# yisol/IDM-VTON

Measured on AMD Instinct MI355X. Metric: try-on images/sec at 768x1024, 30 DDIM steps, guidance 2.0, higher is better.
Workload: dtype bf16; 1 GPU; BASELINE.json configs[1]: 768x1024, 30 steps, batch 2/GPU, guidance 2.0, bf16 storage / fp32 accumulate, scheduler ddim, hipGraph on, GarmentNet batched over 6 timesteps, GarmentNet(block b+1)||TryonNet(block b) two-stream overlap on; images_per_call=2, parallelism=dp1 (image shards, one start-up RCCL weight broadcast), rccl_ranks=1

## Files before the change

### idm-vton_amd/csrc/gemm_body.cuh

```cuda
#pragma once
#include <type_traits>
#if !defined(__gfx950__) && !defined(__gfx942__) && defined(__HIP_DEVICE_COMPILE__)
#error "gemm_body.cuh: the counted vmcnt pipeline is written for gfx94x/gfx950 (stores counted in vmcnt)"
#endif
#include "common.cuh"
#include "gemm_common.cuh"

template <typename T, int BN, int BM, int WN, int WM, int ST, bool V1, bool LIN, bool PF, bool TR, bool XA = false>
__device__ __forceinline__ void gemm_body(const GemmParams& p, char* smem, const int m0, const int n0) {
    typedef typename VT<T>::v8 v8;
    typedef typename VT<T>::v4 v4;
    constexpr int NW = WN * WM;
    constexpr int SN = BN / WN, SM = BM / WM;
    constexpr int NI = SN / 32, MI = SM / 32;
    constexpr int WBYTES = BN * 128, XBYTES = BM * 128;
    constexpr int PW_ = BN / 8, PX_ = BM / 8;
    constexpr bool UNEVEN = (PW_ % NW != 0) || (PX_ % NW != 0);
    constexpr int WI = (PW_ + NW - 1) / NW, XI = (PX_ + NW - 1) / NW;
    static_assert(BN % 8 == 0 && BM % 8 == 0 && WN * SN == BN && WM * SM == BM && NI * 32 == SN && MI * 32 == SM, "tile / wave-count mismatch");
    static_assert(!UNEVEN || (V1 && ST == 2), "round-robin piece assignment needs the two-stage ring");
    char* sW = smem;
    char* sX = smem + ST * WBYTES;

    const int lane = threadIdx.x & 63;
// ... 56 lines not shown
            for (int i = 0; i < XI; ++i) {
                if (UNEVEN && xj(i) >= PX_) continue;
                int iy = x_oy[i] + sg.dy, ix = x_ox[i] + sg.dx;
                const bool ok = (unsigned)iy < (unsigned)hin && (unsigned)ix < (unsigned)win;
                if (p.ups) { iy >>= 1; ix >>= 1; }
                const uint32_t off = ((uint32_t)(x_pix[i] + iy * p.Wi + ix) * (uint32_t)sg.pitch + sg.coff + kseg + x_c8[i]) * 2u;
                dma16(rs_x, dX + xj(i) * 1024, ok ? off : OOB_SENTINEL);
            }
            kseg += 64;
            if (kseg >= sg.len) { kseg = 0; ++si; }
        }
    };

    idmvton_seg sgc = p.seg[0];
    __amdgpu_buffer_rsrc_t rs_xc = rs_x0;
    auto issue_part = [&](int t, int buf, int s) {
        constexpr int LPT_ = WI + XI;
        char* dW = sW + buf * WBYTES;
        char* dX = sX + buf * XBYTES;
        if constexpr (!LIN) {
            if (s == 0) { sgc = p.seg[si]; rs_xc = make_rsrc(sgc.ptr, sgc.bytes); }
        }
#pragma unroll
        for (int j = 0; j < LPT_; ++j) {
            if ((j & 3) != s) continue;
            if (j < WI) {
                if (UNEVEN && wj(j) >= PW_) continue;
                dma16(rs_w, dW + wj(j) * 1024, w_off[j] + kbyte(t));
            } else {
                const int i = j - WI;
                if (UNEVEN && xj(i) >= PX_) continue;
                if constexpr (LIN) dma16(rs_x0, dX + xj(i) * 1024, x_off[i] + kbyte(t));
                else {
                    int iy = x_oy[i] + sgc.dy, ix = x_ox[i] + sgc.dx;
                    const bool ok = (unsigned)iy < (unsigned)hin && (unsigned)ix < (unsigned)win;
                    if (p.ups) { iy >>= 1; ix >>= 1; }
                    const uint32_t off = ((uint32_t)(x_pix[i] + iy * p.Wi + ix) * (uint32_t)sgc.pitch + sgc.coff + kseg + x_c8[i]) * 2u;
                    dma16(rs_xc, dX + xj(i) * 1024, ok ? off : OOB_SENTINEL);
                }
            }
        }
        if constexpr (!LIN) {
            if (s == 3) { kseg += 64; if (kseg >= sgc.len) { kseg = 0; ++si; } }
        }
    };

    int a_row[NI], a_swz[NI], b_row[MI], b_swz[MI];
#pragma unroll
    for (int ni = 0; ni < NI; ++ni) { const int r = wn * SN + ni * 32 + l31; a_row[ni] = r * 128; a_swz[ni] = (r >> 1) & 7; }
#pragma unroll
    for (int mi = 0; mi < MI; ++mi) { const int r = wm * SM + mi * 32 + l31; b_row[mi] = r * 128; b_swz[mi] = (r >> 1) & 7; }

    f32x16 acc[NI][MI];
#pragma unroll
    for (int ni = 0; ni < NI; ++ni)
#pragma unroll
        for (int mi = 0; mi < MI; ++mi)
#pragma unroll
            for (int r = 0; r < 16; ++r) acc[ni][mi][r] = 0.f;

    auto frag_a = [&](const char* bW, int s, int ni) { return *(const v8*)(bW + a_row[ni] + (((2 * s + u) ^ a_swz[ni]) << 4)); };
    auto frag_b = [&](const char* bX, int s, int mi) { return *(const v8*)(bX + b_row[mi] + (((2 * s + u) ^ b_swz[mi]) << 4)); };
    auto compute = [&](int buf, bool spread = false, int t_next = 0, int buf_next = 0) {
        const char* bW = sW + buf * WBYTES;
        const char* bX = sX + buf * XBYTES;
        if constexpr (!PF) {
#pragma unroll
            for (int s = 0; s < 4; ++s) {
                v8 a[NI], b[MI];
#pragma unroll
                for (int ni = 0; ni < NI; ++ni) a[ni] = frag_a(bW, s, ni);
#pragma unroll
                for (int mi = 0; mi < MI; ++mi) b[mi] = frag_b(bX, s, mi);
                if constexpr (V1) {
                    if (spread) issue_part(t_next, buf_next, s);
                    __builtin_amdgcn_sched_barrier(0);
                }
#pragma unroll
                for (int ni = 0; ni < NI; ++ni)
#pragma unroll
                    for (int mi = 0; mi < MI; ++mi)
                        acc[ni][mi] = TR ? VT<T>::mfma(b[mi], a[ni], acc[ni][mi]) : VT<T>::mfma(a[ni], b[mi], acc[ni][mi]);
            }
        } else {
            v8 a[2][NI], b[2][MI];
#pragma unroll
            for (int ni = 0; ni < NI; ++ni) a[0][ni] = frag_a(bW, 0, ni);
#pragma unroll
            for (int mi = 0; mi < MI; ++mi) b[0][mi] = frag_b(bX, 0, mi);
#pragma unroll
            for (int s = 0; s < 4; ++s) {
                if (s < 3) {
#pragma unroll
                    for (int ni = 0; ni < NI; ++ni) a[(s + 1) & 1][ni] = frag_a(bW, s + 1, ni);
#pragma unroll
                    for (int mi = 0; mi < MI; ++mi) b[(s + 1) & 1][mi] = frag_b(bX, s + 1, mi);
                }
                if (spread) issue_part(t_next, buf_next, s);
                __builtin_amdgcn_sched_barrier(0);
#pragma unroll
                for (int ni = 0; ni < NI; ++ni)
#pragma unroll
                    for (int mi = 0; mi < MI; ++mi)
                        acc[ni][mi] = TR ? VT<T>::mfma(b[s & 1][mi], a[s & 1][ni], acc[ni][mi])
                                         : VT<T>::mfma(a[s & 1][ni], b[s & 1][mi], acc[ni][mi]);
                __builtin_amdgcn_sched_barrier(0);
            }
        }
    };

    v8 xkf[XA ? XA_NK : 1];
    int xa_b = 0, xa_h = 0;
    if constexpr (XA) {
        static_assert(NI == 2 && !TR, "fused cross-attention: one 64-channel head per wave");
        const int mw = m0 + wm * SM;
        xa_b = (mw < p.M ? mw : p.M - 1) / p.xa.tokens;
        xa_h = (n0 + wn * SN) >> 6;
        xattn_load_k<T>(p.xa, xa_b, xa_h, lane, xkf);
    }
    const int nt = p.Ktot >> 6;
    if constexpr (!V1) {
        issue(0, 0);
        for (int t = 0; t < nt; ++t) {
            asm volatile("s_waitcnt vmcnt(0)" ::: "memory");
            __syncthreads();
            if (t + 1 < nt) issue(t + 1, (t + 1) & 1);
            compute(t & 1);
        }
    } else {
        constexpr int LPT = WI + XI;
        static_assert((ST - 2) * LPT < 64, "vmcnt immediate is 6 bits");
#pragma unroll
        for (int s = 0; s < ST - 1; ++s)
            if (s < nt) issue(s, s);
        int cbuf = 0, ibuf = ST - 1;
        for (int t = 0; t < nt; ++t) {
            if (t + ST - 2 < nt) wait_vmcnt<(ST - 2) * LPT>(); else wait_vmcnt<0>();
            __builtin_amdgcn_s_barrier();
            asm volatile("" ::: "memory");
            compute(cbuf, t + ST - 1 < nt, t + ST - 1, ibuf);
            cbuf = cbuf + 1 == ST ? 0 : cbuf + 1;
            ibuf = ibuf + 1 == ST ? 0 : ibuf + 1;
        }
    }

    if constexpr (XA) {
        v8 xvf[XA_NV];
        xattn_load_v<T>(p.xa, xa_b, xa_h, lane, xvf);
        xattn_compute<T, MI>(p.xa, p.M, acc, m0 + wm * SM, lane, xkf, xvf);
    }
    gemm_epilogue<T, NI, MI, SN, SM, TR>(p, acc, m0, n0, wn, wm, lane);
}

template <typename T, int BN, int BM, int WN, int WM, int ST, bool V1, bool LIN, int OCC, bool PFX = false>
__global__ __launch_bounds__(WN * WM * 64, OCC) void gemm_conv_kernel(const GemmParams p) {
    __shared__ __attribute__((aligned(1024))) char smem[ST * (BN + BM) * 128];
    const int wg = xcd_remap(blockIdx.x, p.tiles_m * p.tiles_n);
    int tm, tn;
    if constexpr (!V1) { tm = wg / p.tiles_n; tn = wg - tm * p.tiles_n; }
    else {
        const int GM = p.gm > 0 ? p.gm : 1024 / BM;
        const int width = GM * p.tiles_n;
        const int grp = wg / width, rem = wg - grp * width;
        const int first = grp * GM;
        const int gsz = p.tiles_m - first < GM ? p.tiles_m - first : GM;
        tn = rem / gsz; tm = first + (rem - tn * gsz);
    }
    const int m0 = tm * BM, n0 = tn * BN;
    if constexpr (BN == 320) {
        gemm_body<T, BN, BM, WN, WM, ST, V1, LIN, OCC == 1 || PFX, false>(p, smem, m0, n0);
    } else {
        if (p.vt != nullptr && n0 >= p.vt_n0) gemm_body<T, BN, BM, WN, WM, ST, V1, LIN, OCC == 1 || PFX, true>(p, smem, m0, n0);
        else gemm_body<T, BN, BM, WN, WM, ST, V1, LIN, OCC == 1 || PFX, false>(p, smem, m0, n0);
    }
}

template <typename T, int BN, int BM, int WN, int WM, int ST, int OCC>
__global__ __launch_bounds__(WN * WM * 64, OCC) void gemm_xattn_kernel(const GemmParams p) {
    __shared__ __attribute__((aligned(1024))) char smem[ST * (BN + BM) * 128];
    const int wg = xcd_remap(blockIdx.x, p.tiles_m * p.tiles_n);
    const int GM = p.gm > 0 ? p.gm : 1024 / BM;
    const int width = GM * p.tiles_n;
    const int grp = wg / width, rem = wg - grp * width;
    const int first = grp * GM;
    const int gsz = p.tiles_m - first < GM ? p.tiles_m - first : GM;
    const int tn = rem / gsz, tm = first + (rem - tn * gsz);
    gemm_body<T, BN, BM, WN, WM, ST, true, true, OCC == 1, false, true>(p, smem, tm * BM, tn * BN);
}

template <typename T, int BN, int BM, int WN, int WM, int ST, bool V1, int OCC, bool PFX = false>
static void launch_cfg(const GemmParams& p0, bool lin, hipStream_t st) {
    GemmParams p = p0;
    p.gm = V1 ? idmvton_choose_gm(p.tiles_m, p.tiles_n, BM, BN, p.Ktot) : 0;
    const dim3 grid(p.tiles_n * p.tiles_m), block(WN * WM * 64);
    if constexpr (V1) {
        if (lin) { hipLaunchKernelGGL((gemm_conv_kernel<T, BN, BM, WN, WM, ST, true, true, OCC, PFX>), grid, block, 0, st, p); return; }
    }
    hipLaunchKernelGGL((gemm_conv_kernel<T, BN, BM, WN, WM, ST, V1, false, OCC, PFX>), grid, block, 0, st, p);
}


int gemm_tiles_v0(const GemmParams& p, bool bf16, int bn, int bm, bool lin, hipStream_t st);
int gemm_tiles_v1(const GemmParams& p, bool bf16, int bn, int bm, bool lin, hipStream_t st);
int gemm_tiles_v2(const GemmParams& p, bool bf16, int bn, int bm, bool lin, hipStream_t st);
int gemm_tiles_w8(const GemmParams& p, bool bf16, int bn, int bm, int form, bool lin, hipStream_t st);
int gemm_tiles_xattn(const GemmParams& p, bool bf16, int bn, int bm, int w8, hipStream_t st);
int launch_gemm_lin(const GemmParams& p, bool bf16, int bm, int form, int grid_cap, hipStream_t st);
```

### idm-vton_amd/csrc/gemm_common.cuh

```cuda
#pragma once
#include "common.cuh"
#include "xattn.cuh"

struct GemmParams {
    const void* w; uint32_t w_bytes; int N; int Ktot;
    int nseg; idmvton_seg seg[IDMVTON_MAX_SEG];
    int M, Ho, Wo, Hi, Wi, stride, ups;
    void* out; int ldo;
    const void* bias; const void* rowbias; int rowbias_ld; int rows_per_group;
    const void* res; int ldr;
    int mode;
    void* vt; int vt_n0; int vt_tokens; int vt_perm;
    int colscale_n; float colscale;
    int tiles_m, tiles_n;
    int gm;
    int wide;
    int res32, out32;
    int bias32;
    int out8; float o8_scale, vt8_scale;
    XAttnParams xa;
};

int idmvton_choose_gm(int tiles_m, int tiles_n, int bm, int bn, int K);

template <int N> __device__ __forceinline__ void wait_vmcnt() { asm volatile("s_waitcnt vmcnt(%0)" ::"n"(N) : "memory"); }

__device__ __forceinline__ void swap_cols8(const f32x16& c, const int gp, float (&v)[8]) {
#pragma unroll
    for (int j = 0; j < 4; ++j) {
        const auto r = __builtin_amdgcn_permlane32_swap(__float_as_uint(c[8 * gp + j]), __float_as_uint(c[8 * gp + 4 + j]), false, false);
        v[j] = __uint_as_float(r[0]);
        v[4 + j] = __uint_as_float(r[1]);
    }
}

template <typename T, int NI, int MI, int SN, int SM, bool TR>
__device__ __forceinline__ void gemm_epilogue(const GemmParams& p, f32x16 (&acc)[NI][MI], const int m0, const int n0, const int wn, const int wm,
                                              const int lane) {
    typedef typename VT<T>::v4 v4;
    typedef typename VT<T>::v8 v8;
    const int u = lane >> 5, l31 = lane & 31;
    const T* bias = (const T*)p.bias;
    if constexpr (TR) {
        if (p.out8) {
            uint8_t* vt = (uint8_t*)p.vt;
            const int Cv = p.N - p.vt_n0;
#pragma unroll
            for (int ni = 0; ni < NI; ++ni) {
                const int n = n0 + wn * SN + ni * 32 + l31;
                if (n >= p.N) continue;
                const float bv = bias ? (float)bias[n] : 0.f;
#pragma unroll
                for (int mi = 0; mi < MI; ++mi) {
                    const int m = m0 + wm * SM + mi * 32;
                    if (m >= p.M) continue;
                    const int b = m / p.vt_tokens;
                    const int tok = m - b * p.vt_tokens;
                    int4 o;
                    int w[4];
#pragma unroll
                    for (int g = 0; g < 4; ++g)
                        w[g] = pack4_fp8(clamp448((acc[ni][mi][4 * g] + bv) * p.vt8_scale), clamp448((acc[ni][mi][4 * g + 1] + bv) * p.vt8_scale),
                                         clamp448((acc[ni][mi][4 * g + 2] + bv) * p.vt8_scale), clamp448((acc[ni][mi][4 * g + 3] + bv) * p.vt8_scale));
                    o.x = w[0]; o.y = w[1]; o.z = w[2]; o.w = w[3];
                    *(int4*)(vt + ((size_t)(b * Cv + n - p.vt_n0) * p.vt_tokens + (tok & ~63) + 32 * u + ((tok >> 1) & 16))) = o;
                }
            }
            return;
        }
        if (p.vt_perm) {
            T* vt = (T*)p.vt;
            const int Cv = p.N - p.vt_n0;
#pragma unroll
            for (int ni = 0; ni < NI; ++ni) {
                const int n = n0 + wn * SN + ni * 32 + l31;
                if (n >= p.N) continue;
                const float bv = bias ? (float)bias[n] : 0.f;
#pragma unroll
                for (int mi = 0; mi < MI; ++mi)
#pragma unroll
                    for (int gp = 0; gp < 2; ++gp) {
                        const int m = m0 + wm * SM + mi * 32 + 16 * gp;
                        if (m >= p.M) continue;
                        const int b = m / p.vt_tokens;
                        const int tok = m - b * p.vt_tokens + 8 * u;
                        v8 o;
#pragma unroll
                        for (int j = 0; j < 8; ++j) o[j] = (T)(acc[ni][mi][8 * gp + j] + bv);
                        *(v8*)(vt + ((size_t)(b * Cv + n - p.vt_n0) * p.vt_tokens + tok)) = o;
                    }
            }
            return;
        }
        T* vt = (T*)p.vt;
        const int Cv = p.N - p.vt_n0;
#pragma unroll
        for (int ni = 0; ni < NI; ++ni) {
            const int n = n0 + wn * SN + ni * 32 + l31;
            if (n >= p.N) continue;
            const float bv = bias ? (float)bias[n] : 0.f;
#pragma unroll
            for (int mi = 0; mi < MI; ++mi)
#pragma unroll
                for (int g = 0; g < 4; ++g) {
                    const int m = m0 + wm * SM + mi * 32 + 8 * g + 4 * u;
                    if (m >= p.M) continue;
                    const int b = m / p.vt_tokens;
                    int tok = m - b * p.vt_tokens;
                    if (p.vt_perm) tok = (tok & ~12) | ((tok & 4) << 1) | ((tok & 8) >> 1);
                    v4 o;
#pragma unroll
                    for (int j = 0; j < 4; ++j) o[j] = (T)(acc[ni][mi][4 * g + j] + bv);
                    *(v4*)(vt + ((size_t)(b * Cv + n - p.vt_n0) * p.vt_tokens + tok)) = o;
                }
        }
        return;
    }
    T* out = (T*)p.out;
    const T* res = (const T*)p.res;
    const T* rowbias = (const T*)p.rowbias;
    if (p.wide) {
#pragma unroll
        for (int mi = 0; mi < MI; ++mi) {
            const int m = m0 + wm * SM + mi * 32 + l31;
            if (m >= p.M) continue;
            const T* rb = rowbias ? rowbias + (size_t)(m / p.rows_per_group) * p.rowbias_ld : nullptr;
            if (p.mode == IDMVTON_EPI_GEGLU) {
                if constexpr (NI % 2 == 0) {
#pragma unroll
                    for (int pr = 0; pr < NI / 2; ++pr)
#pragma unroll
                        for (int gp = 0; gp < 2; ++gp) {
                            float h[8], gt[8];
                            swap_cols8(acc[2 * pr][mi], gp, h);
                            swap_cols8(acc[2 * pr + 1][mi], gp, gt);
                            const int nh = n0 + wn * SN + pr * 64 + 16 * gp + 8 * u;
                            if (nh + 32 >= p.N) continue;
                            const int jo = ((n0 + wn * SN + pr * 64) >> 1) + 16 * gp + 8 * u;
                            if (bias) {
                                const v8 bh = *(const v8*)(bias + nh), bg = *(const v8*)(bias + nh + 32);
#pragma unroll
                                for (int j = 0; j < 8; ++j) { h[j] += (float)bh[j]; gt[j] += (float)bg[j]; }
                            }
                            v8 o;
#pragma unroll
                            for (int j = 0; j < 8; ++j) o[j] = (T)(h[j] * gelu_erf(gt[j]));
                            *(v8*)(out + (size_t)m * p.ldo + jo) = o;
                        }
                }
                continue;
            }
#pragma unroll
            for (int ni = 0; ni < NI; ++ni) {
#pragma unroll
                for (int gp = 0; gp < 2; ++gp) {
                    float v[8];
                    swap_cols8(acc[ni][mi], gp, v);
                    const int n = n0 + wn * SN + ni * 32 + 16 * gp + 8 * u;
                    if (n >= p.N) continue;
                    if (bias) {
                        if (p.bias32) {
                            const float4* bp = (const float4*)((const float*)p.bias + n);
                            const float4 b0 = bp[0], b1 = bp[1];
                            v[0] += b0.x; v[1] += b0.y; v[2] += b0.z; v[3] += b0.w;
                            v[4] += b1.x; v[5] += b1.y; v[6] += b1.z; v[7] += b1.w;
                        } else {
                            const v8 bb = *(const v8*)(bias + n);
#pragma unroll
                            for (int j = 0; j < 8; ++j) v[j] += (float)bb[j];
                        }
                    }
                    if (rb) {
// ... 120 lines not shown
```

### idm-vton_amd/csrc/gemm_conv.hip

```cpp
#include <cstdlib>
#include <cstring>
#include <vector>
#include "gemm_body.cuh"

int launch_gemm_lin(const GemmParams& p, bool bf16, int bm, int form, int grid_cap, hipStream_t st);

#include <map>
#include <mutex>
#include <tuple>
int idmvton_choose_gm(int tiles_m, int tiles_n, int bm, int bn, int K) {
    static const char* env = getenv("IDMVTON_GM");
    if (env) return atoi(env);
    static const bool model = getenv("IDMVTON_GM_MODEL") && atoi(getenv("IDMVTON_GM_MODEL")) != 0;
    if (!model) return 0;
    static std::mutex mu;
    static std::map<std::tuple<int, int, int, int, int>, int> cache;
    const auto key = std::make_tuple(tiles_m, tiles_n, bm, bn, K);
    std::lock_guard<std::mutex> lk(mu);
    auto it = cache.find(key);
    if (it != cache.end()) return it->second;
    const int T = tiles_m * tiles_n, q = T / 8, r = T % 8;
    static const long cap = getenv("IDMVTON_GM_CAP_KB") ? atol(getenv("IDMVTON_GM_CAP_KB")) << 10 : (2l << 20);
    long best = -1; int best_gm = 0;
    for (int gm = 1; gm <= tiles_m; ++gm) {
// ... 12 lines not shown
                if (!ns[tn]) { ns[tn] = 1; ++cn; }
            }
            (void)m_lo; (void)m_hi;
            cost += (long)cm * bm + (long)cn * bn;
        }
        if (best < 0 || cost < best) { best = cost; best_gm = gm; }
    }
    cache[key] = best_gm;
    return best_gm;
}

static int launch_gemm(const GemmParams& p0, bool bf16, int variant, int bn, int bm, bool lin, hipStream_t st) {
    GemmParams p = p0;
    int form = 0;
    int grid_cap = 0;
    if (variant == 5) { form = bm & 15; grid_cap = (bm & 0x4000) ? 5 : 0; bm &= ~(15 | 0x4000); }
    p.tiles_n = (p.N + bn - 1) / bn;
    p.tiles_m = (p.M + bm - 1) / bm;
    int rc = 1;
    if (p.mode == IDMVTON_EPI_XATTN) {
        if (bm != 64 && p.xa.tokens % 64 != 0) {
            bm = 64;
            p.tiles_m = (p.M + bm - 1) / bm;
        }
        if (gemm_tiles_xattn(p, bf16, bn, bm, variant == 6 && bn == 128 && bm == 128, st))
            return idmvton_set_error(IDMVTON_E_ARG, "gemm_conv: IDMVTON_EPI_XATTN runs on the 128x64, 128x128 and 128x256 tiles (got %dx%d)", bn, bm);
        CHECK_LAUNCH("gemm_conv");
        return IDMVTON_OK;
    }
    if (variant == 0) rc = gemm_tiles_v0(p, bf16, bn, bm, lin, st);
    else if (variant == 1) rc = gemm_tiles_v1(p, bf16, bn, bm, lin, st);
    else if (variant == 2) rc = gemm_tiles_v2(p, bf16, bn, bm, lin, st);
    else if (variant == 5) {
        if (!(bn == 256 && (bm == 256 || bm == 192))) return idmvton_set_error(IDMVTON_E_ARG, "gemm_conv: variant 5 is the 256x256 / 256x192 tile");
        if (lin) rc = launch_gemm_lin(p, bf16, bm, form, grid_cap, st);
        else if (bm == 256) rc = gemm_tiles_v1(p, bf16, 256, 256, lin, st);
        else {
            p.tiles_n = (p.N + 127) / 128; p.tiles_m = (p.M + 255) / 256;
            rc = gemm_tiles_v1(p, bf16, 128, 256, lin, st);
        }
    } else if (variant == 6) {
        const int form6 = bm & 15;
        bm &= ~15;
        p.tiles_m = (p.M + bm - 1) / bm;
        if (bn == 320 && (p.vt || !p.wide || p.out8 || p.mode == IDMVTON_EPI_GEGLU)) {
            const int fbn = bn == 320 ? 128 : bn, fbm = bn == 320 ? 256 : bm;
            p.tiles_n = (p.N + fbn - 1) / fbn;
            p.tiles_m = (p.M + fbm - 1) / fbm;
            rc = gemm_tiles_v1(p, bf16, fbn, fbm, lin, st);
        } else rc = gemm_tiles_w8(p, bf16, bn, bm, form6, lin, st);
    } else return idmvton_set_error(IDMVTON_E_ARG, "gemm_conv: unknown variant %d", variant);
    if (rc) return idmvton_set_error(IDMVTON_E_ARG, "gemm_conv: variant %d has no %dx%d tile", variant, bn, bm);
    CHECK_LAUNCH("gemm_conv");
    return IDMVTON_OK;
}

extern "C" int idmvton_gemm_conv(const idmvton_gemm_conv_args* a, void* stream) {
    CHECK_ARG(a != nullptr, IDMVTON_E_ARG, "gemm_conv: null args");
    CHECK_ARG(a->dtype == IDMVTON_F16 || a->dtype == IDMVTON_BF16, IDMVTON_E_DTYPE, "gemm_conv: dtype %d", a->dtype);
    CHECK_ARG(a->M > 0 && a->N > 0 && a->Ktot > 0, IDMVTON_E_SHAPE, "gemm_conv: M=%d N=%d K=%d", a->M, a->N, a->Ktot);
    CHECK_ARG(a->Ktot % 64 == 0, IDMVTON_E_SHAPE, "gemm_conv: Ktot=%d must be a multiple of 64", a->Ktot);
    CHECK_ARG(a->N % 4 == 0, IDMVTON_E_SHAPE, "gemm_conv: N=%d must be a multiple of 4", a->N);
    CHECK_ARG(a->nseg >= 1 && a->nseg <= IDMVTON_MAX_SEG, IDMVTON_E_SHAPE, "gemm_conv: nseg=%d", a->nseg);
    int ksum = 0;
    for (int s = 0; s < a->nseg; ++s) {
        const idmvton_seg& g = a->seg[s];
        CHECK_ARG(g.ptr && g.len > 0 && g.len % 64 == 0, IDMVTON_E_SHAPE, "gemm_conv: seg %d len=%d", s, g.len);
        CHECK_ARG(g.pitch % 8 == 0 && g.coff % 8 == 0, IDMVTON_E_ALIGN, "gemm_conv: seg %d pitch=%d coff=%d", s, g.pitch, g.coff);
        CHECK_ARG(g.bytes < 0x80000000u, IDMVTON_E_SHAPE, "gemm_conv: seg %d tensor >= 2 GiB", s);
        CHECK_ARG(((uintptr_t)g.ptr & 15) == 0, IDMVTON_E_ALIGN, "gemm_conv: seg %d pointer not 16-byte aligned", s);
        ksum += g.len;
    }
    CHECK_ARG(ksum == a->Ktot, IDMVTON_E_SHAPE, "gemm_conv: segment lengths sum to %d, Ktot=%d", ksum, a->Ktot);
    CHECK_ARG(a->Ho > 0 && a->Wo > 0 && a->Hi > 0 && a->Wi > 0 && a->stride > 0 && a->M % (a->Ho * a->Wo) == 0,
              IDMVTON_E_SHAPE, "gemm_conv: geometry M=%d Ho=%d Wo=%d", a->M, a->Ho, a->Wo);
    if (a->ups) CHECK_ARG(a->stride == 1 && a->Ho <= 2 * a->Hi && a->Ho >= 2 * a->Hi - 1 && a->Wo <= 2 * a->Wi && a->Wo >= 2 * a->Wi - 1, IDMVTON_E_SHAPE,
                          "gemm_conv: ups=1 needs stride 1 and an output grid of 2Hi x 2Wi or one short of it (Ho=%d Hi=%d Wo=%d Wi=%d)", a->Ho, a->Hi, a->Wo, a->Wi);
    CHECK_ARG(a->w && ((uintptr_t)a->w & 15) == 0, IDMVTON_E_ALIGN, "gemm_conv: weight pointer");
    const uint64_t wbytes = (uint64_t)a->N * a->Ktot * 2;
    CHECK_ARG(wbytes + (uint64_t)128 * a->Ktot * 2 < 0xFFFFFFFFull, IDMVTON_E_SHAPE, "gemm_conv: weight too large");
    const bool geglu = a->mode == IDMVTON_EPI_GEGLU, xattn = a->mode == IDMVTON_EPI_XATTN;
    CHECK_ARG(a->mode == IDMVTON_EPI_NONE || a->mode == IDMVTON_EPI_GELU || a->mode == IDMVTON_EPI_QUICKGELU || geglu || xattn, IDMVTON_E_ARG, "gemm_conv: mode %d", a->mode);
    CHECK_ARG(a->colscale_n >= 0 && a->colscale_n % 4 == 0 && !(geglu && a->colscale_n), IDMVTON_E_ARG, "gemm_conv: colscale_n=%d", a->colscale_n);
    if (geglu) CHECK_ARG(a->N % 64 == 0 && !a->res && !a->rowbias && !a->vt, IDMVTON_E_ARG, "gemm_conv: GEGLU needs N%%64==0, no res/rowbias/vt");
    CHECK_ARG(a->out || (a->vt && a->vt_n0 == 0), IDMVTON_E_ARG, "gemm_conv: null out");
    if (a->out) CHECK_ARG(a->ldo % 4 == 0 && ((uintptr_t)a->out & 7) == 0, IDMVTON_E_ALIGN, "gemm_conv: out alignment");
    if (a->res) CHECK_ARG(a->ldr % 4 == 0 && ((uintptr_t)a->res & 7) == 0, IDMVTON_E_ALIGN, "gemm_conv: res alignment");
    if (a->bias) CHECK_ARG(((uintptr_t)a->bias & 7) == 0, IDMVTON_E_ALIGN, "gemm_conv: bias alignment");
    if (a->rowbias) CHECK_ARG(a->rowbias_ld % 4 == 0 && a->rows_per_group > 0 && ((uintptr_t)a->rowbias & 7) == 0,
                              IDMVTON_E_ALIGN, "gemm_conv: rowbias");
    if (a->vt && a->vt_perm) CHECK_ARG(((uintptr_t)a->vt & 15) == 0, IDMVTON_E_ALIGN, "gemm_conv: vt pointer not 16-byte aligned");
    if (a->vt && a->vt_perm) CHECK_ARG(a->vt_tokens % 16 == 0, IDMVTON_E_ARG, "gemm_conv: vt_perm needs vt_tokens %% 16 == 0 (got %d)", a->vt_tokens);
    if (a->vt) CHECK_ARG(a->vt_tokens > 0 && a->vt_tokens % 4 == 0 && a->M % a->vt_tokens == 0 && a->vt_n0 % 64 == 0 &&
                         a->vt_n0 >= 0 && a->vt_n0 < a->N && ((uintptr_t)a->vt & 7) == 0,
                         IDMVTON_E_ARG, "gemm_conv: vt_tokens=%d vt_n0=%d", a->vt_tokens, a->vt_n0);

    GemmParams p;
    memset(&p.xa, 0, sizeof(p.xa));
    if (xattn) {
        const idmvton_xattn* x = a->xattn;
        CHECK_ARG(x != nullptr && (x->nseg == 1 || x->nseg == 2), IDMVTON_E_ARG, "gemm_conv: IDMVTON_EPI_XATTN needs `xattn` with 1 or 2 key segments");
        CHECK_ARG(a->N % 64 == 0 && !a->bias && !a->res && !a->rowbias && !a->vt && !a->colscale_n && !a->io_flags &&
                  a->nseg == 1 && a->Ho == 1 && a->Hi == 1 && a->Wo == a->M && a->Wi == a->M && a->out && a->ldo % 8 == 0 && ((uintptr_t)a->out & 15) == 0,
                  IDMVTON_E_ARG, "gemm_conv: IDMVTON_EPI_XATTN is a plain Linear with N %% 64 == 0 and nothing else in its epilogue");
        CHECK_ARG(x->tokens > 0 && x->tokens % 32 == 0 && a->M % x->tokens == 0, IDMVTON_E_SHAPE, "gemm_conv: xattn.tokens=%d (rows per batch element, a multiple of 32 dividing M=%d)", x->tokens, a->M);
        for (int s = 0; s < x->nseg; ++s) {
            const int nk_max = s == 0 ? 96 : 32;
            CHECK_ARG(x->k[s] && x->vt[s] && x->nk[s] > 0 && x->nk[s] <= nk_max && x->k_rows[s] >= ((x->nk[s] + 31) & ~31) && x->ldk[s] >= a->N && x->ldk[s] % 8 == 0 &&
                      x->ldvt[s] >= ((x->nk[s] + 15) & ~15) && x->ldvt[s] % 8 == 0 && (((uintptr_t)x->k[s] | (uintptr_t)x->vt[s]) & 15) == 0, IDMVTON_E_SHAPE,
                      "gemm_conv: xattn segment %d: nk=%d (<= %d) k_rows=%d (>= round32(nk)) ldk=%d ldvt=%d (>= round16(nk))", s, x->nk[s], nk_max, x->k_rows[s], x->ldk[s], x->ldvt[s]);
            p.xa.k[s] = x->k[s]; p.xa.vt[s] = x->vt[s]; p.xa.ldk[s] = x->ldk[s]; p.xa.ldvt[s] = x->ldvt[s]; p.xa.nk[s] = x->nk[s]; p.xa.krows[s] = x->k_rows[s];
        }
        p.xa.nseg = x->nseg; p.xa.tokens = x->tokens; p.xa.vchan = a->N; p.xa.ip_scale = x->ip_scale;
    } else CHECK_ARG(a->xattn == nullptr, IDMVTON_E_ARG, "gemm_conv: `xattn` without mode IDMVTON_EPI_XATTN");
    p.w = a->w; p.w_bytes = (uint32_t)wbytes; p.N = a->N; p.Ktot = a->Ktot;
    p.nseg = a->nseg;
    for (int s = 0; s < IDMVTON_MAX_SEG; ++s) p.seg[s] = a->seg[s < a->nseg ? s : a->nseg - 1];
    p.M = a->M; p.Ho = a->Ho; p.Wo = a->Wo; p.Hi = a->Hi; p.Wi = a->Wi; p.stride = a->stride; p.ups = a->ups ? 1 : 0;
    p.out = a->out; p.ldo = a->ldo; p.bias = a->bias; p.rowbias = a->rowbias; p.rowbias_ld = a->rowbias_ld;
    p.rows_per_group = a->rows_per_group > 0 ? a->rows_per_group : 1; p.res = a->res; p.ldr = a->ldr; p.mode = a->mode;
    p.vt = a->vt; p.vt_n0 = a->vt_n0; p.vt_tokens = a->vt_tokens > 0 ? a->vt_tokens : 4; p.vt_perm = a->vt_perm ? 1 : 0;
    p.colscale_n = a->colscale_n; p.colscale = a->colscale;
    p.tiles_m = p.tiles_n = 0; p.gm = 0;
    {
        auto a16 = [](const void* q) { return ((uintptr_t)q & 15) == 0; };
        const int n_out = geglu ? a->N / 2 : a->N;
        p.wide = n_out % 8 == 0 && a->N % 8 == 0 && a->colscale_n % 8 == 0 && (!a->out || (a->ldo % 8 == 0 && a16(a->out))) &&
                 (!a->res || (a->ldr % 8 == 0 && a16(a->res))) && (!a->bias || a16(a->bias)) &&
                 (!a->rowbias || (a->rowbias_ld % 8 == 0 && a16(a->rowbias))) && (!a->vt || a->vt_n0 % 8 == 0);
    }

    int variant = 1, bn = 64, bm = 64;
    static const bool env_narrow = getenv("IDMVTON_EPILOGUE_8B") != nullptr;
    if ((a->tile_hint & 0x8000) || env_narrow) p.wide = 0;
    p.res32 = (a->io_flags & IDMVTON_IO_RES_F32) ? 1 : 0;
    p.out32 = (a->io_flags & IDMVTON_IO_OUT_F32) ? 1 : 0;
    p.bias32 = (a->io_flags & IDMVTON_IO_BIAS_F32) ? 1 : 0;
    if (p.bias32) CHECK_ARG(a->bias && p.wide && !geglu && !a->vt && ((uintptr_t)a->bias & 15) == 0, IDMVTON_E_ARG,
                            "gemm_conv: IDMVTON_IO_BIAS_F32 needs a 16-byte aligned bias and the plain 16-byte epilogue (no GEGLU, no vt)");
    CHECK_ARG((a->io_flags & ~15) == 0, IDMVTON_E_ARG, "gemm_conv: io_flags=%d", a->io_flags);
    p.out8 = (a->io_flags & IDMVTON_IO_OUT_F8) ? 1 : 0;
    p.o8_scale = a->f8_out_scale; p.vt8_scale = a->f8_vt_scale;
    if (p.out8) {
        CHECK_ARG(a->io_flags == IDMVTON_IO_OUT_F8 && a->mode == IDMVTON_EPI_NONE && !a->res && !a->rowbias && p.wide,
                  IDMVTON_E_ARG, "gemm_conv: IDMVTON_IO_OUT_F8 needs the plain 16-byte epilogue (no activation / residual / rowbias / fp32 IO)");
        CHECK_ARG((!a->out || a->f8_out_scale > 0.f) && (!a->vt || (a->f8_vt_scale > 0.f && a->vt_tokens % 64 == 0 && ((uintptr_t)a->vt & 15) == 0)),
                  IDMVTON_E_ARG, "gemm_conv: IDMVTON_IO_OUT_F8: scales > 0, vt_tokens %% 64 == 0 (got %d), 16-byte aligned vt", a->vt_tokens);
    }
    if (p.res32 || p.out32) {
        CHECK_ARG((a->io_flags & ~7) == 0 && !geglu && !a->vt, IDMVTON_E_ARG, "gemm_conv: io_flags=%d (fp32 res / out: no GEGLU, no vt)", a->io_flags);
        CHECK_ARG(!p.res32 || a->res, IDMVTON_E_ARG, "gemm_conv: IDMVTON_IO_RES_F32 without res");
        CHECK_ARG(p.wide, IDMVTON_E_ALIGN, "gemm_conv: the fp32 residual stream needs the 16-byte epilogue (N, ldo, ldr multiples of 8, 16-byte aligned pointers)");
    }
    if (a->tile_hint) { variant = (a->tile_hint >> 28) & 0xf; bn = (a->tile_hint >> 16) & 0xfff; bm = a->tile_hint & 0x7fff; }
    else {
        static const int cand[5][2] = {{256, 256}, {128, 256}, {128, 128}, {128, 64}, {64, 64}};
        for (int i = 0; i < 5; ++i) {
            const int n_ = cand[i][0], m_ = cand[i][1];
            if (geglu && n_ < 128) continue;
            if (xattn && (n_ != 128)) continue;
            if (a->vt && a->vt_n0 % n_ != 0) continue;
            if (i < 4 && (n_ > ((a->N + 63) & ~63) || m_ > ((a->M + 63) & ~63))) continue;
            bn = n_; bm = m_;
            if ((long)((a->N + n_ - 1) / n_) * ((a->M + m_ - 1) / m_) >= 200) break;
        }
    }
    if (geglu) CHECK_ARG(bn >= 128, IDMVTON_E_ARG, "gemm_conv: GEGLU needs BN >= 128 (64-row wave tiles)");
    if (a->vt) CHECK_ARG(a->vt_n0 % bn == 0, IDMVTON_E_ARG, "gemm_conv: vt_n0 %% BN != 0");
    const idmvton_seg& s0 = a->seg[0];
    const bool lin = a->nseg == 1 && a->Ho == 1 && a->Hi == 1 && a->Wo == a->M && a->Wi == a->M && a->stride == 1 &&
                     !a->ups && s0.dy == 0 && s0.dx == 0 && (uint64_t)a->M * s0.pitch * 2 < 0x80000000ull;
    if (!a->tile_hint && bn == 256 && bm == 256 && lin) { variant = 5; bm = 257; }
    else if (!a->tile_hint && !xattn) {
        if (bn == 256 && bm == 256) variant = 6;
        else if (bn == 128 && bm == 128) variant = 6;
        if (a->N > 256 && a->N <= 320 && p.wide && !a->vt && !geglu && !p.out8 && (a->M + 191) / 192 >= 200) { variant = 6; bn = 320; bm = 192; }
    }
    hipStream_t st = (hipStream_t)stream;
    return launch_gemm(p, a->dtype == IDMVTON_BF16, variant, bn, bm, lin, st);
}
```

### idm-vton_amd/csrc/gemm_tiles_v1.hip

```cpp
#include "gemm_body.cuh"

template <typename T>
static int run(const GemmParams& p, int bn, int bm, bool lin, hipStream_t st) {
    if (bn == 256 && bm == 256) launch_cfg<T, 256, 256, 2, 4, 2, true, 2>(p, lin, st);
    else if (bn == 128 && bm == 256) launch_cfg<T, 128, 256, 2, 4, 3, true, 2>(p, lin, st);
    else if (bn == 128 && bm == 128) launch_cfg<T, 128, 128, 2, 2, 3, true, 1>(p, lin, st);
    else if (bn == 128 && bm == 64) launch_cfg<T, 128, 64, 2, 2, 3, true, 2>(p, lin, st);
    else if (bn == 64 && bm == 64) launch_cfg<T, 64, 64, 2, 2, 4, true, 2>(p, lin, st);
    else return 1;
    return 0;
}
int gemm_tiles_v1(const GemmParams& p, bool bf16, int bn, int bm, bool lin, hipStream_t st) {
    return bf16 ? run<bf16_t>(p, bn, bm, lin, st) : run<f16_t>(p, bn, bm, lin, st);
}
```

### idm-vton_amd/csrc/gemm_tiles_v2.hip

```cpp
#include "gemm_body.cuh"

template <typename T>
static int run(const GemmParams& p, int bn, int bm, bool lin, hipStream_t st) {
    if (bn == 128 && bm == 256) launch_cfg<T, 128, 256, 2, 4, 3, true, 2, true>(p, lin, st);
    else if (bn == 64 && bm == 64) launch_cfg<T, 64, 64, 2, 2, 4, true, 2, true>(p, lin, st);
    else return 1;
    return 0;
}
int gemm_tiles_v2(const GemmParams& p, bool bf16, int bn, int bm, bool lin, hipStream_t st) {
    return bf16 ? run<bf16_t>(p, bn, bm, lin, st) : run<f16_t>(p, bn, bm, lin, st);
}
```

### idm-vton_amd/csrc/gemm_tiles_w8.hip

```cpp
#include "gemm_body.cuh"

template <typename T>
static int run(const GemmParams& p, int bn, int bm, int form, bool lin, hipStream_t st) {
    if (bn == 128 && bm == 128 && form == 0) launch_cfg<T, 128, 128, 2, 4, 3, true, 2>(p, lin, st);
    else if (bn == 128 && bm == 128 && form == 1) launch_cfg<T, 128, 128, 2, 4, 3, true, 2, true>(p, lin, st);
    else if (bn == 320 && bm == 192) launch_cfg<T, 320, 192, 2, 6, 2, true, 3>(p, lin, st);
    else if (bn == 256 && bm == 192) launch_cfg<T, 256, 192, 4, 3, 2, true, 3>(p, lin, st);
    else if (bn == 256 && bm == 256) launch_cfg<T, 256, 256, 4, 4, 2, true, 4>(p, lin, st);
    else if (bn == 128 && bm == 256) launch_cfg<T, 128, 256, 2, 8, 3, true, 4>(p, lin, st);
    else return 1;
    return 0;
}
int gemm_tiles_w8(const GemmParams& p, bool bf16, int bn, int bm, int form, bool lin, hipStream_t st) {
    return bf16 ? run<bf16_t>(p, bn, bm, form, lin, st) : run<f16_t>(p, bn, bm, form, lin, st);
}
```

Before: 1.641 images/s.

## Add row-slab 3x3 conv loader reusing activation rows across dx taps

Adds a gemm_body_slab path for stride-1 3x3 convolutions detected from the 9-segment layout. It loads one activation row slab (BM+2 rows) per dy and channel chunk into LDS and reuses it across the three dx taps with masked boundary fragments, instead of reloading the activation tile for each tap. This is meant to cut global and LDS traffic for the implicit-GEMM conv. It adds a three-slab LDS ring and a new synchronisation schedule, and can be disabled through an env var or a hint bit.

```diff
diff --git a/idm-vton_amd/csrc/conv_sets.h b/idm-vton_amd/csrc/conv_sets.h
--- /dev/null
+++ b/idm-vton_amd/csrc/conv_sets.h
@@ -0,0 +1,54 @@
+#pragma once
+#include <stdint.h>
+#include "../../include/idmvton_hip.h"
+
+#define IDMVTON_MAX_CONV_SETS 3
+
+typedef struct {
+    int32_t seg;
+    int32_t kbase;
+    int32_t ktap;
+    int32_t len;
+} idmvton_conv_set;
+
+static inline int idmvton_conv_sets_detect(const idmvton_seg* seg, int nseg, int stride, int ups, int Ho, int Wo, int Hi, int Wi,
+                                           idmvton_conv_set* out) {
+    if (seg == nullptr || out == nullptr) return 0;
+    if (stride != 1 || ups || Ho != Hi || Wo != Wi || Hi <= 0 || Wi <= 0) return 0;
+    if (nseg < 9 || nseg > IDMVTON_MAX_SEG || nseg % 9 != 0 || nseg / 9 > IDMVTON_MAX_CONV_SETS) return 0;
+    int nsets = 0;
+    int seen[IDMVTON_MAX_CONV_SETS];
+    int koff[IDMVTON_MAX_CONV_SETS][9];
+    int k = 0;
+    for (int i = 0; i < nseg; ++i) {
+        const idmvton_seg& g = seg[i];
+        if (g.len <= 0 || g.len % 64 != 0) return 0;
+        if (g.dy < -1 || g.dy > 1 || g.dx < -1 || g.dx > 1) return 0;
+        int s = 0;
+        for (; s < nsets; ++s) {
+            const idmvton_seg& h = seg[out[s].seg];
+            if (h.ptr == g.ptr && h.bytes == g.bytes && h.pitch == g.pitch && h.coff == g.coff && h.len == g.len) break;
+        }
+        if (s == nsets) {
+            if (nsets == IDMVTON_MAX_CONV_SETS) return 0;
+            out[s].seg = i; out[s].len = g.len; out[s].kbase = 0; out[s].ktap = 0;
+            seen[s] = 0;
+            ++nsets;
+        }
+        const int tap = (g.dy + 1) * 3 + (g.dx + 1);
+        if (seen[s] & (1 << tap)) return 0;
+        seen[s] |= 1 << tap;
+        koff[s][tap] = k;
+        k += g.len;
+    }
+    if (nsets * 9 != nseg) return 0;
+    for (int s = 0; s < nsets; ++s) {
+        if (seen[s] != 0x1ff) return 0;
+        out[s].kbase = koff[s][0];
+        out[s].ktap = koff[s][1] - koff[s][0];
+        if (out[s].ktap < out[s].len) return 0;
+        for (int tap = 0; tap < 9; ++tap)
+            if (koff[s][tap] != out[s].kbase + tap * out[s].ktap) return 0;
+    }
+    return nsets;
+}
diff --git a/idm-vton_amd/csrc/gemm_body.cuh b/idm-vton_amd/csrc/gemm_body.cuh
--- a/idm-vton_amd/csrc/gemm_body.cuh
+++ b/idm-vton_amd/csrc/gemm_body.cuh
@@ -232,6 +232,240 @@
     gemm_epilogue<T, NI, MI, SN, SM, TR>(p, acc, m0, n0, wn, wm, lane);
 }
 
+template <typename T, int BN, int BM, int WN, int WM, int ST, bool PF>
+__device__ __forceinline__ void gemm_body_slab(const GemmParams& p, char* smem, const int m0, const int n0) {
+    typedef typename VT<T>::v8 v8;
+    constexpr int NW = WN * WM;
+    constexpr int SN = BN / WN, SM = BM / WM;
+    constexpr int NI = SN / 32, MI = SM / 32;
+    constexpr int WBYTES = BN * 128;
+    constexpr int SP = BM / 8 + 1, SBYTES = SP * 1024;
+    constexpr int PW_ = BN / 8;
+    constexpr bool UNEVEN = PW_ % NW != 0;
+    constexpr int WI = (PW_ + NW - 1) / NW;
+    constexpr int XS = (SP + 3 * NW - 1) / (3 * NW);
+    constexpr int XP = (SP + NW - 1) / NW;
+    constexpr int LPT = WI + XS;
+    static_assert((ST == 2 || ST == 3) && (!UNEVEN || ST == 2) && NW % 2 == 0 && BM % 8 == 0 && WN * SN == BN && WM * SM == BM && NI * 32 == SN && MI * 32 == SM, "tile / wave-count mismatch");
+    static_assert(LPT < 64, "vmcnt immediate is 6 bits");
+    char* sW = smem;
+    char* sS = smem + ST * WBYTES;
+    char* sPad = sS + 3 * SBYTES;
+
+    const int lane = threadIdx.x & 63;
+    const int wave = uniform(threadIdx.x >> 6);
+    const int wn = wave / WM, wm = wave % WM;
+    const int u = lane >> 5, l31 = lane & 31;
+    const int lrow = lane >> 3, lslot = lane & 7;
+
+    auto wj = [&](int i) { return UNEVEN ? wave + i * NW : wave * WI + i; };
+    uint32_t w_off[WI];
+#pragma unroll
+    for (int i = 0; i < WI; ++i) {
+        const int R = wj(i) * 8 + lrow;
+        const int c = lslot ^ ((R >> 1) & 7);
+        w_off[i] = ((uint32_t)(n0 + R) * (uint32_t)p.Ktot + c * 8) * 2u;
+    }
+    const __amdgpu_buffer_rsrc_t rs_w = make_rsrc(p.w, p.w_bytes);
+
+    const int jq = wave * 8 + lrow;
+    const int qb = m0 - 1 + jq;
+    const uint32_t c8b = (uint32_t)((lslot ^ (((wave & 1) << 2) | (lrow >> 1))) * 16);
+
+    int cur_s = 0, cur_dy = -1, cur_c0 = 0;
+    GemmSlabSet cs = p.sset[0];
+    __amdgpu_buffer_rsrc_t s_rs = make_rsrc(cs.ptr, cs.bytes);
+    uint32_t s_pitch2 = (uint32_t)cs.pitch * 2u, s_add = 0, w_k0 = 0, w_kstep = 0;
+    int s_dq = 0, s_qlim = 0, w_dy = -1;
+    auto derive_slab = [&]() {
+        s_add = (uint32_t)(cs.coff + cur_c0) * 2u;
+        s_dq = cur_dy * p.Wi;
+        s_qlim = cur_s < p.nsets ? p.M : 0;
+    };
+    auto step = [&]() {
+        w_k0 = (uint32_t)(cs.kbase + (cur_dy + 1) * 3 * cs.ktap + cur_c0) * 2u;
+        w_kstep = (uint32_t)cs.ktap * 2u;
+        w_dy = cur_dy;
+        cur_c0 += 64;
+        if (cur_c0 >= cs.len) {
+            cur_c0 = 0;
+            if (++cur_dy == 2) {
+                cur_dy = -1;
+                ++cur_s;
+                cs = p.sset[cur_s < p.nsets ? cur_s : p.nsets - 1];
+                s_rs = make_rsrc(cs.ptr, cs.bytes);
+                s_pitch2 = (uint32_t)cs.pitch * 2u;
+            }
+        }
+        derive_slab();
+    };
+    auto slab_dma = [&](char* sbuf, int pc_rel) {
+        const int pc = pc_rel + wave;
+        if (ST == 2 && pc >= SP) return;
+        const int j = jq + pc_rel * 8;
+        const int q = qb + pc_rel * 8 + s_dq;
+        const bool ok = j < BM + 2 && (unsigned)q < (unsigned)s_qlim;
+        const uint32_t off = (uint32_t)q * s_pitch2 + s_add + c8b;
+        dma16(s_rs, pc < SP ? sbuf + pc * 1024 : sPad, ok ? off : OOB_SENTINEL);
+    };
+    auto issue_set = [&](int dxi, int h, int wbuf, char* sbuf, int part) {
+        char* dW = sW + wbuf * WBYTES;
+        const uint32_t kb = w_k0 + (uint32_t)dxi * w_kstep;
+#pragma unroll
+        for (int j = 0; j < LPT; ++j) {
+            if (part >= 0 && (j & 3) != part) continue;
+            if (j < WI) {
+                if (UNEVEN && wj(j) >= PW_) continue;
+                dma16(rs_w, dW + wj(j) * 1024, w_off[j] + kb);
+            } else slab_dma(sbuf, (h * XS + (j - WI)) * NW);
+        }
+    };
+
+    int a_row[NI], a_swz[NI], b_row[MI], b_swz[MI][3], vmask[MI];
+#pragma unroll
+    for (int ni = 0; ni < NI; ++ni) { const int r = wn * SN + ni * 32 + l31; a_row[ni] = r * 128; a_swz[ni] = (r >> 1) & 7; }
+    const int HW = p.Hi * p.Wi;
+#pragma unroll
+    for (int mi = 0; mi < MI; ++mi) {
+        const int r = wm * SM + mi * 32 + l31;
+        b_row[mi] = r * 128;
+#pragma unroll
+        for (int d = 0; d < 3; ++d) b_swz[mi][d] = ((r + d) >> 1) & 7;
+        const int m = m0 + r;
+        int mask = 0;
+        if (m < p.M) {
+            const int b = m / HW, rem = m - b * HW;
+            const int oy = rem / p.Wi, ox = rem - oy * p.Wi;
+#pragma unroll
+            for (int t = 0; t < 9; ++t)
+                if ((unsigned)(oy + t / 3 - 1) < (unsigned)p.Hi && (unsigned)(ox + t % 3 - 1) < (unsigned)p.Wi) mask |= 1 << t;
+        }
+        vmask[mi] = mask;
+    }
+
+    f32x16 acc[NI][MI];
+#pragma unroll
+    for (int ni = 0; ni < NI; ++ni)
+#pragma unroll
+        for (int mi = 0; mi < MI; ++mi)
+#pragma unroll
+            for (int r = 0; r < 16; ++r) acc[ni][mi][r] = 0.f;
+
+    auto frag_a = [&](const char* bW, int s, int ni) { return *(const v8*)(bW + a_row[ni] + (((2 * s + u) ^ a_swz[ni]) << 4)); };
+    auto frag_b = [&](const char* bS, int s, int mi, int dxi) { return *(const v8*)(bS + b_row[mi] + dxi * 128 + (((2 * s + u) ^ b_swz[mi][dxi]) << 4)); };
+    auto compute = [&](int wbuf, const char* bS, int dxi, int bit, auto&& part) {
+        const char* bW = sW + wbuf * WBYTES;
+        bool keep[MI];
+        const v8 zero = {};
+#pragma unroll
+        for (int mi = 0; mi < MI; ++mi) keep[mi] = (vmask[mi] >> bit) & 1;
+        if constexpr (!PF) {
+#pragma unroll
+            for (int s = 0; s < 4; ++s) {
+                v8 a[NI], b[MI];
+#pragma unroll
+                for (int ni = 0; ni < NI; ++ni) a[ni] = frag_a(bW, s, ni);
+#pragma unroll
+                for (int mi = 0; mi < MI; ++mi) b[mi] = frag_b(bS, s, mi, dxi);
+                part(s);
+                __builtin_amdgcn_sched_barrier(0);
+#pragma unroll
+                for (int mi = 0; mi < MI; ++mi) b[mi] = keep[mi] ? b[mi] : zero;
+#pragma unroll
+                for (int ni = 0; ni < NI; ++ni)
+#pragma unroll
+                    for (int mi = 0; mi < MI; ++mi) acc[ni][mi] = VT<T>::mfma(a[ni], b[mi], acc[ni][mi]);
+            }
+        } else {
+            v8 a[2][NI], b[2][MI];
+#pragma unroll
+            for (int ni = 0; ni < NI; ++ni) a[0][ni] = frag_a(bW, 0, ni);
+#pragma unroll
+            for (int mi = 0; mi < MI; ++mi) b[0][mi] = frag_b(bS, 0, mi, dxi);
+#pragma unroll
+            for (int s = 0; s < 4; ++s) {
+                if (s < 3) {
+#pragma unroll
+                    for (int ni = 0; ni < NI; ++ni) a[(s + 1) & 1][ni] = frag_a(bW, s + 1, ni);
+#pragma unroll
+                    for (int mi = 0; mi < MI; ++mi) b[(s + 1) & 1][mi] = frag_b(bS, s + 1, mi, dxi);
+                }
+                part(s);
+                __builtin_amdgcn_sched_barrier(0);
+#pragma unroll
+                for (int mi = 0; mi < MI; ++mi) b[s & 1][mi] = keep[mi] ? b[s & 1][mi] : zero;
+#pragma unroll
+                for (int ni = 0; ni < NI; ++ni)
+#pragma unroll
+                    for (int mi = 0; mi < MI; ++mi) acc[ni][mi] = VT<T>::mfma(a[s & 1][ni], b[s & 1][mi], acc[ni][mi]);
+                __builtin_amdgcn_sched_barrier(0);
+            }
+        }
+    };
+
+    const int ng = p.Ktot / 192;
+    if constexpr (ST == 3) {
+        derive_slab();
+    #pragma unroll
+        for (int k = 0; k < XP; ++k) slab_dma(sS, k * NW);
+        step();
+        issue_set(0, 0, 0, sS + SBYTES, -1);
+        issue_set(1, 1, 1, sS + SBYTES, -1);
+        int so_r = 0, so_a = SBYTES, so_b = 2 * SBYTES;
+        int r_dy = -1;
+        for (int g = 0; g < ng; ++g) {
+            const bool more = g + 1 < ng;
+            const int bit0 = (r_dy + 1) * 3;
+            wait_vmcnt<LPT>();
+            __builtin_amdgcn_s_barrier();
+            asm volatile("" ::: "memory");
+            compute(0, sS + so_r, 0, bit0, [&](int s) { issue_set(2, 2, 2, sS + so_a, s); });
+            step();
+            wait_vmcnt<LPT>();
+            __builtin_amdgcn_s_barrier();
+            asm volatile("" ::: "memory");
+            compute(1, sS + so_r, 1, bit0 + 1, [&](int s) { if (more) issue_set(0, 0, 0, sS + so_b, s); });
+            if (more) wait_vmcnt<LPT>(); else wait_vmcnt<0>();
+            __builtin_amdgcn_s_barrier();
+            asm volatile("" ::: "memory");
+            compute(2, sS + so_r, 2, bit0 + 2, [&](int s) { if (more) issue_set(1, 1, 1, sS + so_b, s); });
+            r_dy = w_dy;
+            const int so_t = so_r; so_r = so_a; so_a = so_b; so_b = so_t;
+        }
+    } else {
+        derive_slab();
+#pragma unroll
+        for (int k = 0; k < XP; ++k) slab_dma(sS, k * NW);
+        step();
+        issue_set(0, 0, 0, sS + SBYTES, -1);
+        int so_r = 0, so_a = SBYTES, so_b = 2 * SBYTES;
+        int r_dy = -1, t = 0;
+        for (int g = 0; g < ng; ++g) {
+            const bool more = g + 1 < ng;
+            const int bit0 = (r_dy + 1) * 3;
+            wait_vmcnt<0>();
+            __builtin_amdgcn_s_barrier();
+            asm volatile("" ::: "memory");
+            compute(t & 1, sS + so_r, 0, bit0, [&](int s) { issue_set(1, 1, (t + 1) & 1, sS + so_a, s); });
+            ++t;
+            wait_vmcnt<0>();
+            __builtin_amdgcn_s_barrier();
+            asm volatile("" ::: "memory");
+            compute(t & 1, sS + so_r, 1, bit0 + 1, [&](int s) { issue_set(2, 2, (t + 1) & 1, sS + so_a, s); });
+            ++t;
+            step();
+            wait_vmcnt<0>();
+            __builtin_amdgcn_s_barrier();
+            asm volatile("" ::: "memory");
+            compute(t & 1, sS + so_r, 2, bit0 + 2, [&](int s) { if (more) issue_set(0, 0, (t + 1) & 1, sS + so_b, s); });
+            ++t;
+            r_dy = w_dy;
+            const int so_t = so_r; so_r = so_a; so_a = so_b; so_b = so_t;
+        }
+    }
+    gemm_epilogue<T, NI, MI, SN, SM, false>(p, acc, m0, n0, wn, wm, lane);
+}
+
 template <typename T, int BN, int BM, int WN, int WM, int ST, bool V1, bool LIN, int OCC, bool PFX = false>
 __global__ __launch_bounds__(WN * WM * 64, OCC) void gemm_conv_kernel(const GemmParams p) {
     __shared__ __attribute__((aligned(1024))) char smem[ST * (BN + BM) * 128];
@@ -268,11 +502,29 @@
     gemm_body<T, BN, BM, WN, WM, ST, true, true, OCC == 1, false, true>(p, smem, tm * BM, tn * BN);
 }
 
-template <typename T, int BN, int BM, int WN, int WM, int ST, bool V1, int OCC, bool PFX = false>
+template <typename T, int BN, int BM, int WN, int WM, int ST, int OCC, bool PFX>
+__global__ __launch_bounds__(WN * WM * 64, OCC) void gemm_conv_slab_kernel(const GemmParams p) {
+    __shared__ __attribute__((aligned(1024))) char smem[ST * BN * 128 + 3 * (BM / 8 + 1) * 1024 + 1024];
+    static_assert(sizeof(smem) <= 160 * 1024, "LDS budget");
+    const int wg = xcd_remap(blockIdx.x, p.tiles_m * p.tiles_n);
+    const int GM = p.gm > 0 ? p.gm : 1024 / BM;
+    const int width = GM * p.tiles_n;
+    const int grp = wg / width, rem = wg - grp * width;
+    const int first = grp * GM;
+    const int gsz = p.tiles_m - first < GM ? p.tiles_m - first : GM;
+    const int tn = rem / gsz, tm = first + (rem - tn * gsz);
+    gemm_body_slab<T, BN, BM, WN, WM, ST, OCC == 1 || PFX>(p, smem, tm * BM, tn * BN);
+}
+
+template <typename T, int BN, int BM, int WN, int WM, int ST, bool V1, int OCC, bool PFX = false, bool SLAB = false>
 static void launch_cfg(const GemmParams& p0, bool lin, hipStream_t st) {
     GemmParams p = p0;
     p.gm = V1 ? idmvton_choose_gm(p.tiles_m, p.tiles_n, BM, BN, p.Ktot) : 0;
     const dim3 grid(p.tiles_n * p.tiles_m), block(WN * WM * 64);
+    if constexpr (SLAB) {
+        static_assert(V1 && (ST == 2 || ST == 3), "the row-slab loader rides the two- or three-stage ring");
+        if (!lin && p.nsets > 0) { hipLaunchKernelGGL((gemm_conv_slab_kernel<T, BN, BM, WN, WM, ST, OCC, PFX>), grid, block, 0, st, p); return; }
+    }
     if constexpr (V1) {
         if (lin) { hipLaunchKernelGGL((gemm_conv_kernel<T, BN, BM, WN, WM, ST, true, true, OCC, PFX>), grid, block, 0, st, p); return; }
     }
diff --git a/idm-vton_amd/csrc/gemm_common.cuh b/idm-vton_amd/csrc/gemm_common.cuh
--- a/idm-vton_amd/csrc/gemm_common.cuh
+++ b/idm-vton_amd/csrc/gemm_common.cuh
@@ -1,6 +1,9 @@
 #pragma once
 #include "common.cuh"
 #include "xattn.cuh"
+#include "conv_sets.h"
+
+struct GemmSlabSet { const void* ptr; uint32_t bytes; int32_t pitch, coff, len, kbase, ktap; };
 
 struct GemmParams {
     const void* w; uint32_t w_bytes; int N; int Ktot;
@@ -18,6 +21,7 @@
     int res32, out32;
     int bias32;
     int out8; float o8_scale, vt8_scale;
+    int nsets; GemmSlabSet sset[IDMVTON_MAX_CONV_SETS];
     XAttnParams xa;
 };
 
diff --git a/idm-vton_amd/csrc/gemm_conv.hip b/idm-vton_amd/csrc/gemm_conv.hip
--- a/idm-vton_amd/csrc/gemm_conv.hip
+++ b/idm-vton_amd/csrc/gemm_conv.hip
@@ -188,7 +188,20 @@
         CHECK_ARG(!p.res32 || a->res, IDMVTON_E_ARG, "gemm_conv: IDMVTON_IO_RES_F32 without res");
         CHECK_ARG(p.wide, IDMVTON_E_ALIGN, "gemm_conv: the fp32 residual stream needs the 16-byte epilogue (N, ldo, ldr multiples of 8, 16-byte aligned pointers)");
     }
-    if (a->tile_hint) { variant = (a->tile_hint >> 28) & 0xf; bn = (a->tile_hint >> 16) & 0xfff; bm = a->tile_hint & 0x7fff; }
+    static const bool env_taps = getenv("IDMVTON_CONV_TAPS") != nullptr && atoi(getenv("IDMVTON_CONV_TAPS")) != 0;
+    const int hint = a->tile_hint & ~0x2000;
+    p.nsets = 0;
+    memset(p.sset, 0, sizeof(p.sset));
+    if (!xattn && !a->vt && !env_taps && !(a->tile_hint & 0x2000)) {
+        idmvton_conv_set cs[IDMVTON_MAX_CONV_SETS];
+        p.nsets = idmvton_conv_sets_detect(a->seg, a->nseg, a->stride, a->ups ? 1 : 0, a->Ho, a->Wo, a->Hi, a->Wi, cs);
+        for (int s = 0; s < p.nsets; ++s) {
+            const idmvton_seg& g = a->seg[cs[s].seg];
+            p.sset[s].ptr = g.ptr; p.sset[s].bytes = g.bytes; p.sset[s].pitch = g.pitch; p.sset[s].coff = g.coff;
+            p.sset[s].len = cs[s].len; p.sset[s].kbase = cs[s].kbase; p.sset[s].ktap = cs[s].ktap;
+        }
+    }
+    if (hint) { variant = (hint >> 28) & 0xf; bn = (hint >> 16) & 0xfff; bm = hint & 0x7fff; }
     else {
         static const int cand[5][2] = {{256, 256}, {128, 256}, {128, 128}, {128, 64}, {64, 64}};
         for (int i = 0; i < 5; ++i) {
@@ -206,8 +219,8 @@
     const idmvton_seg& s0 = a->seg[0];
     const bool lin = a->nseg == 1 && a->Ho == 1 && a->Hi == 1 && a->Wo == a->M && a->Wi == a->M && a->stride == 1 &&
                      !a->ups && s0.dy == 0 && s0.dx == 0 && (uint64_t)a->M * s0.pitch * 2 < 0x80000000ull;
-    if (!a->tile_hint && bn == 256 && bm == 256 && lin) { variant = 5; bm = 257; }
-    else if (!a->tile_hint && !xattn) {
+    if (!hint && bn == 256 && bm == 256 && lin) { variant = 5; bm = 257; }
+    else if (!hint && !xattn) {
         if (bn == 256 && bm == 256) variant = 6;
         else if (bn == 128 && bm == 128) variant = 6;
         if (a->N > 256 && a->N <= 320 && p.wide && !a->vt && !geglu && !p.out8 && (a->M + 191) / 192 >= 200) { variant = 6; bn = 320; bm = 192; }
diff --git a/idm-vton_amd/csrc/gemm_tiles_v1.hip b/idm-vton_amd/csrc/gemm_tiles_v1.hip
--- a/idm-vton_amd/csrc/gemm_tiles_v1.hip
+++ b/idm-vton_amd/csrc/gemm_tiles_v1.hip
@@ -3,8 +3,8 @@
 template <typename T>
 static int run(const GemmParams& p, int bn, int bm, bool lin, hipStream_t st) {
     if (bn == 256 && bm == 256) launch_cfg<T, 256, 256, 2, 4, 2, true, 2>(p, lin, st);
-    else if (bn == 128 && bm == 256) launch_cfg<T, 128, 256, 2, 4, 3, true, 2>(p, lin, st);
-    else if (bn == 128 && bm == 128) launch_cfg<T, 128, 128, 2, 2, 3, true, 1>(p, lin, st);
+    else if (bn == 128 && bm == 256) launch_cfg<T, 128, 256, 2, 4, 3, true, 2, false, true>(p, lin, st);
+    else if (bn == 128 && bm == 128) launch_cfg<T, 128, 128, 2, 2, 3, true, 1, false, true>(p, lin, st);
     else if (bn == 128 && bm == 64) launch_cfg<T, 128, 64, 2, 2, 3, true, 2>(p, lin, st);
     else if (bn == 64 && bm == 64) launch_cfg<T, 64, 64, 2, 2, 4, true, 2>(p, lin, st);
     else return 1;
diff --git a/idm-vton_amd/csrc/gemm_tiles_v2.hip b/idm-vton_amd/csrc/gemm_tiles_v2.hip
--- a/idm-vton_amd/csrc/gemm_tiles_v2.hip
+++ b/idm-vton_amd/csrc/gemm_tiles_v2.hip
@@ -2,7 +2,7 @@
 
 template <typename T>
 static int run(const GemmParams& p, int bn, int bm, bool lin, hipStream_t st) {
-    if (bn == 128 && bm == 256) launch_cfg<T, 128, 256, 2, 4, 3, true, 2, true>(p, lin, st);
+    if (bn == 128 && bm == 256) launch_cfg<T, 128, 256, 2, 4, 3, true, 2, true, true>(p, lin, st);
     else if (bn == 64 && bm == 64) launch_cfg<T, 64, 64, 2, 2, 4, true, 2, true>(p, lin, st);
     else return 1;
     return 0;
diff --git a/idm-vton_amd/csrc/gemm_tiles_w8.hip b/idm-vton_amd/csrc/gemm_tiles_w8.hip
--- a/idm-vton_amd/csrc/gemm_tiles_w8.hip
+++ b/idm-vton_amd/csrc/gemm_tiles_w8.hip
@@ -2,12 +2,12 @@
 
 template <typename T>
 static int run(const GemmParams& p, int bn, int bm, int form, bool lin, hipStream_t st) {
-    if (bn == 128 && bm == 128 && form == 0) launch_cfg<T, 128, 128, 2, 4, 3, true, 2>(p, lin, st);
-    else if (bn == 128 && bm == 128 && form == 1) launch_cfg<T, 128, 128, 2, 4, 3, true, 2, true>(p, lin, st);
-    else if (bn == 320 && bm == 192) launch_cfg<T, 320, 192, 2, 6, 2, true, 3>(p, lin, st);
-    else if (bn == 256 && bm == 192) launch_cfg<T, 256, 192, 4, 3, 2, true, 3>(p, lin, st);
+    if (bn == 128 && bm == 128 && form == 0) launch_cfg<T, 128, 128, 2, 4, 3, true, 2, false, true>(p, lin, st);
+    else if (bn == 128 && bm == 128 && form == 1) launch_cfg<T, 128, 128, 2, 4, 3, true, 2, true, true>(p, lin, st);
+    else if (bn == 320 && bm == 192) launch_cfg<T, 320, 192, 2, 6, 2, true, 3, false, true>(p, lin, st);
+    else if (bn == 256 && bm == 192) launch_cfg<T, 256, 192, 4, 3, 2, true, 3, false, true>(p, lin, st);
     else if (bn == 256 && bm == 256) launch_cfg<T, 256, 256, 4, 4, 2, true, 4>(p, lin, st);
-    else if (bn == 128 && bm == 256) launch_cfg<T, 128, 256, 2, 8, 3, true, 4>(p, lin, st);
+    else if (bn == 128 && bm == 256) launch_cfg<T, 128, 256, 2, 8, 3, true, 4, false, true>(p, lin, st);
     else return 1;
     return 0;
 }
```

Result: no change. 1.656 images/s, median of 6 (+0.9%).
